# rlawhdrhs/Vision-Transformer-OpenCL

Measured on AMD Instinct MI355X. Metric: images/sec ViT-B/16 224² fp32 @batch256; % MFMA roofline; top-1 match, higher is better.
Workload: dtype f32; 1 GPU; ViT-B/16 224x224 fp32 forward, batch 256 per GPU, synthetic weights and images (BASELINE.json configs[1]); batch_per_gpu=256, global_batch=256, parallelism=dp1, lanes_per_gpu=1, prune_last_layer=False, ln_fold=True, device=AMD Radeon Graphics, arch=gfx950:sramecc+:xnack-, compute_units=256, clock_mhz=2400

## Files before the change

### vision-transformer-opencl_amd/csrc/vit_attention_hd.hip

```cpp
#include <hip/hip_runtime.h>

#include <math.h>

#include <type_traits>

#include "vit_attention.hpp"
#include "vit_hip_kernels.h"
#include "vit_split3.hpp"

namespace {

using namespace vitattn;
typedef unsigned int u32x2 __attribute__((ext_vector_type(2)));

constexpr int HD_WAVES = 4, HD_THREADS = HD_WAVES * 64;
constexpr int HD_QROWS = HD_WAVES * 32;

template <int HD, bool BF16>
struct Geo {
    typedef typename std::conditional<BF16, bf16_t, float>::type elem;
    static constexpr int VEC = BF16 ? 8 : 4;
    static constexpr int KC = BF16 ? 64 : 32;
    static constexpr int KT = KC / 32;
    static constexpr int DT = (HD + 31) / 32;
    static constexpr int HDK = BF16 ? (HD + 15) / 16 * 16 : HD;
    static constexpr int KROW = HDK + (BF16 ? 8 : 4);
    static constexpr int VROW = KC + 4;
    static constexpr int K_ELEMS = KC * KROW, V_ELEMS = DT * 32 * VROW;
    static constexpr int MIN_WAVES = BF16 && HD <= 96 ? 4 : 3;
};

template <int HD, bool BF16, bool QS>
__global__ __launch_bounds__(HD_THREADS, (Geo<HD, BF16>::MIN_WAVES)) void attention_hd_kernel(
    const typename Geo<HD, BF16>::elem *__restrict__ qkv, typename Geo<HD, BF16>::elem *__restrict__ out, int tokens, int heads, int q_rows,
    int qblocks, float scale) {
    typedef Geo<HD, BF16> G;
    typedef typename G::elem elem;
    constexpr int VEC = G::VEC, KC = G::KC, KT = G::KT, DT = G::DT, KROW = G::KROW, VROW = G::VROW;
    __shared__ __attribute__((aligned(16))) elem Ks[G::K_ELEMS];
    __shared__ __attribute__((aligned(16))) elem Vt[G::V_ELEMS];

    const int tid = threadIdx.x, lane = tid & 63, wave = tid >> 6;
    const int r = lane & 31, h = lane >> 5;
    const int image = blockIdx.x / qblocks, qblock = blockIdx.x - image * qblocks, head = blockIdx.y;
    const size_t D = (size_t)heads * HD, ld = 3 * D;
    const elem *rows = qkv + (size_t)image * tokens * ld + (size_t)head * HD;
    const elem *krows = rows + D, *vrows = rows + 2 * D;
    const int qrow0 = qblock * HD_QROWS + wave * 32;
    const bool active = qrow0 < q_rows;

    constexpr int NQ = BF16 ? G::HDK / 16 : HD / 8;
    typename std::conditional<BF16, bf16x8, f32x4>::type qf[NQ];
    {
        int qrow = qrow0 + r;
        qrow = qrow < q_rows ? qrow : q_rows - 1;
        const elem *qp = rows + (size_t)qrow * ld;
#pragma unroll
        for (int ks = 0; ks < NQ; ++ks) {
            if constexpr (BF16) {
                const int d0 = 16 * ks + 8 * h;
                u32x4 w = {0u, 0u, 0u, 0u};
                if (d0 < HD && active) w = *reinterpret_cast<const u32x4 *>(qp + d0);
                qf[ks] = __builtin_bit_cast(bf16x8, w);
            } else {
                f32x4 w = {0.0f, 0.0f, 0.0f, 0.0f};
                if (active) w = *reinterpret_cast<const f32x4 *>(qp + 8 * ks + 4 * h);
                qf[ks] = w;
            }
        }
    }

    f32x16 o[DT];
#pragma unroll
    for (int dt = 0; dt < DT; ++dt)
#pragma unroll
        for (int v = 0; v < 16; ++v) o[dt][v] = 0.0f;
    float m_run = -INFINITY, l_run = 0.0f;

    for (int key0 = 0; key0 < tokens; key0 += KC) {
        constexpr int KP = G::HDK / VEC;
        for (int i = tid; i < KC * KP; i += HD_THREADS) {
            const int row = i / KP, c = i - row * KP, key = key0 + row;
            u32x4 w = {0u, 0u, 0u, 0u};
            if (key < tokens && c * VEC < HD) w = *reinterpret_cast<const u32x4 *>(krows + (size_t)key * ld + c * VEC);
            *reinterpret_cast<u32x4 *>(Ks + row * KROW + c * VEC) = w;
        }
        constexpr int VP = HD / VEC;
        if constexpr (BF16) {
            for (int i = tid; i < (KC / 2) * VP; i += HD_THREADS) {
                const int c = i / (KC / 2), row = 2 * (i - c * (KC / 2)), key = key0 + row;
                u32x4 a = {0u, 0u, 0u, 0u}, b = {0u, 0u, 0u, 0u};
                if (key < tokens) a = *reinterpret_cast<const u32x4 *>(vrows + (size_t)key * ld + c * VEC);
                if (key + 1 < tokens) b = *reinterpret_cast<const u32x4 *>(vrows + (size_t)(key + 1) * ld + c * VEC);
#pragma unroll
                for (int j = 0; j < 4; ++j) {
                    *reinterpret_cast<unsigned *>(Vt + (c * 8 + 2 * j) * VROW + row) = (a[j] & 0xffffu) | (b[j] << 16);
                    *reinterpret_cast<unsigned *>(Vt + (c * 8 + 2 * j + 1) * VROW + row) = (a[j] >> 16) | (b[j] & 0xffff0000u);
                }
            }
        } else {
            for (int i = tid; i < KC * VP; i += HD_THREADS) {
                const int c = i / KC, row = i - c * KC, key = key0 + row;
                u32x4 w = {0u, 0u, 0u, 0u};
                if (key < tokens) w = *reinterpret_cast<const u32x4 *>(vrows + (size_t)key * ld + c * VEC);
#pragma unroll
                for (int j = 0; j < 4; ++j) Vt[(c * 4 + j) * VROW + row] = __uint_as_float(w[j]);
            }
        }
        __syncthreads();

        if (active) {
#pragma unroll
            for (int t = 0; t < KT; ++t) {
                const int tile0 = key0 + 32 * t;
                if (tile0 >= tokens) break;
                f32x16 s;
#pragma unroll
                for (int v = 0; v < 16; ++v) s[v] = 0.0f;
                const elem *kp = Ks + (32 * t + r) * KROW;
#pragma unroll
                for (int ks = 0; ks < NQ; ++ks) {
                    if constexpr (BF16) {
                        const bf16x8 kf = *reinterpret_cast<const bf16x8 *>(kp + 16 * ks + 8 * h);
                        s = __builtin_amdgcn_mfma_f32_32x32x16_bf16(kf, qf[ks], s, 0, 0, 0);
                    } else {
                        const f32x4 kf = *reinterpret_cast<const f32x4 *>(kp + 8 * ks + 4 * h);
#pragma unroll
                        for (int i = 0; i < 4; ++i) s = __builtin_amdgcn_mfma_f32_32x32x2f32(kf[i], qf[ks][i], s, 0, 0, 0);
                    }
                }
                if (tile0 + 32 > tokens) {
#pragma unroll
                    for (int v = 0; v < 16; ++v) {
                        const int key = tile0 + (v & 3) + 8 * (v >> 2) + 4 * h;
                        s[v] = key < tokens ? s[v] : -INFINITY;
                    }
                }
                float cmax = s[0];
#pragma unroll
                for (int v = 1; v < 16; ++v) cmax = fmaxf(cmax, s[v]);
                cmax = fmaxf(cmax, __shfl_xor(cmax, 32));
                constexpr float kDefer = 8.0f;
                const float m_old = m_run;
                const float m_new = (cmax - m_old) * scale > kDefer ? cmax : m_old;
                const float mneg = -m_new * scale;
                m_run = m_new;
                float sum = 0.0f;
#pragma unroll
                for (int v = 0; v < 16; ++v) {
                    s[v] = __builtin_amdgcn_exp2f(QS ? s[v] + mneg : fmaf(s[v], scale, mneg));
                    sum += s[v];
                }
                if (__any(m_new != m_old)) {
                    const float alpha = __builtin_amdgcn_exp2f((m_old - m_new) * scale);
                    l_run *= alpha;
#pragma unroll
                    for (int dt = 0; dt < DT; ++dt)
#pragma unroll
                        for (int v = 0; v < 16; ++v) o[dt][v] *= alpha;
                }
                l_run += sum;
                if constexpr (BF16) {
#pragma unroll
                    for (int s2 = 0; s2 < 2; ++s2) {
                        bf16x8 pf, pl;
#pragma unroll
                        for (int j = 0; j < 8; ++j) {
                            pf[j] = (__bf16)s[8 * s2 + j];
                            pl[j] = (__bf16)(s[8 * s2 + j] - (float)pf[j]);
                        }
#pragma unroll
                        for (int dt = 0; dt < DT; ++dt) {
                            const bf16_t *vp = Vt + (32 * dt + r) * VROW + 32 * t + 16 * s2 + 4 * h;
                            const u32x2 lo = *reinterpret_cast<const u32x2 *>(vp), hi = *reinterpret_cast<const u32x2 *>(vp + 8);
                            const u32x4 both = {lo[0], lo[1], hi[0], hi[1]};
                            o[dt] = __builtin_amdgcn_mfma_f32_32x32x16_bf16(__builtin_bit_cast(bf16x8, both), pl, o[dt], 0, 0, 0);
                            o[dt] = __builtin_amdgcn_mfma_f32_32x32x16_bf16(__builtin_bit_cast(bf16x8, both), pf, o[dt], 0, 0, 0);
                        }
                    }
                } else {
#pragma unroll
                    for (int q = 0; q < 4; ++q)
#pragma unroll
                        for (int dt = 0; dt < DT; ++dt) {
                            const f32x4 vf = *reinterpret_cast<const f32x4 *>(Vt + (32 * dt + r) * VROW + 32 * t + 8 * q + 4 * h);
#pragma unroll
                            for (int i = 0; i < 4; ++i) o[dt] = __builtin_amdgcn_mfma_f32_32x32x2f32(vf[i], s[4 * q + i], o[dt], 0, 0, 0);
                        }
                }
            }
        }
        __syncthreads();
    }

    const int qrow = qrow0 + r;
    if (active && qrow < q_rows) {
        const float inv = 1.0f / (l_run + __shfl_xor(l_run, 32));
        elem *dst = out + ((size_t)image * tokens + qrow) * D + (size_t)head * HD;
#pragma unroll
        for (int dt = 0; dt < DT; ++dt)
#pragma unroll
            for (int q = 0; q < 4; ++q) {
                const int d0 = 32 * dt + 8 * q + 4 * h;
                if (d0 < HD) {
                    if constexpr (BF16) {
                        bf16x4 w;
#pragma unroll
                        for (int i = 0; i < 4; ++i) w[i] = (__bf16)(o[dt][4 * q + i] * inv);
                        *reinterpret_cast<u32x2 *>(dst + d0) = __builtin_bit_cast(u32x2, w);
                    } else {
                        const f32x4 w = {o[dt][4 * q] * inv, o[dt][4 * q + 1] * inv, o[dt][4 * q + 2] * inv, o[dt][4 * q + 3] * inv};
                        *reinterpret_cast<f32x4 *>(dst + d0) = w;
                    }
                }
            }
    }
}

#ifndef ATT_SPLIT_WAVES
#define ATT_SPLIT_WAVES 4
#endif
#ifndef ATT_SPLIT_MINW
#define ATT_SPLIT_MINW 3
#endif
constexpr int SP_WAVES = ATT_SPLIT_WAVES, SP_THREADS = SP_WAVES * 64, SP_QROWS = SP_WAVES * 32;

__global__ __launch_bounds__(SP_THREADS, ATT_SPLIT_MINW) void attention_split_kernel(const float *__restrict__ qkv, float *__restrict__ out,
                                                                                    int tokens, int heads, int q_rows, int qblocks) {
    using vitsplit::SPLIT_TERM_A;
    using vitsplit::SPLIT_TERM_W;
    using vitsplit::split3_piece8;
    typedef Geo<64, true> G;
    constexpr int HD = 64, KC = G::KC, KT = G::KT, DT = G::DT, KROW = G::KROW, VROW = G::VROW, NQ = HD / 16;
    __shared__ __attribute__((aligned(16))) bf16_t Ks[3 * G::K_ELEMS];
    __shared__ __attribute__((aligned(16))) bf16_t Vt[3 * G::V_ELEMS];

    const int tid = threadIdx.x, lane = tid & 63, wave = tid >> 6;
    const int r = lane & 31, h = lane >> 5;
    const int image = blockIdx.x / qblocks, qblock = blockIdx.x - image * qblocks, head = blockIdx.y;
    const size_t D = (size_t)heads * HD, ld = 3 * D;
    const float *rows = qkv + (size_t)image * tokens * ld + (size_t)head * HD;
    const float *krows = rows + D, *vrows = rows + 2 * D;
    const int qrow0 = qblock * SP_QROWS + wave * 32;
    const bool active = qrow0 < q_rows;
    const f32x4 zero4 = {0.0f, 0.0f, 0.0f, 0.0f};

    bf16x8 qf[3][NQ];
    {
        int qrow = qrow0 + r;
        qrow = qrow < q_rows ? qrow : q_rows - 1;
        const float *qp = rows + (size_t)qrow * ld + 8 * h;
#pragma unroll
        for (int ks = 0; ks < NQ; ++ks) {
            f32x4 x0 = zero4, x1 = zero4;
            if (active) {
                x0 = *reinterpret_cast<const f32x4 *>(qp + 16 * ks);
                x1 = *reinterpret_cast<const f32x4 *>(qp + 16 * ks + 4);
            }
#pragma unroll
            for (int pl = 0; pl < 3; ++pl) qf[pl][ks] = __builtin_bit_cast(bf16x8, split3_piece8(x0, x1, pl));
        }
    }

    f32x16 o[DT];
#pragma unroll
    for (int dt = 0; dt < DT; ++dt)
#pragma unroll
        for (int v = 0; v < 16; ++v) o[dt][v] = 0.0f;
    float m_run = -INFINITY, l_run = 0.0f;

    constexpr int K_ITEMS = KC * (HD / 8), V_ITEMS = (KC / 2) * (HD / 8);
    constexpr int KI = (K_ITEMS + SP_THREADS - 1) / SP_THREADS;
    constexpr int V_TID0 = SP_THREADS > V_ITEMS ? SP_THREADS - V_ITEMS : 0;
    static_assert(V_ITEMS <= SP_THREADS, "one V item per thread at most");
    const int vi = tid - V_TID0;
    f32x4 kx[KI][2], vx[4];
    auto fetch = [&](int key0) {
#pragma unroll
        for (int it = 0; it < KI; ++it) {
            const int i = tid + it * SP_THREADS, row = i / (HD / 8), c = i - row * (HD / 8), key = key0 + row;
            kx[it][0] = kx[it][1] = zero4;
            if (i < K_ITEMS && key < tokens) {
                const float *p = krows + (size_t)key * ld + 8 * c;
                kx[it][0] = *reinterpret_cast<const f32x4 *>(p);
                kx[it][1] = *reinterpret_cast<const f32x4 *>(p + 4);
            }
        }
        if (vi >= 0) {
            const int c = vi / (KC / 2), key = key0 + 2 * (vi - c * (KC / 2));
#pragma unroll
            for (int j = 0; j < 4; ++j) vx[j] = zero4;
            if (key < tokens) {
                const float *p = vrows + (size_t)key * ld + 8 * c;
                vx[0] = *reinterpret_cast<const f32x4 *>(p);
                vx[1] = *reinterpret_cast<const f32x4 *>(p + 4);
            }
            if (key + 1 < tokens) {
                const float *p = vrows + (size_t)(key + 1) * ld + 8 * c;
                vx[2] = *reinterpret_cast<const f32x4 *>(p);
                vx[3] = *reinterpret_cast<const f32x4 *>(p + 4);
            }
        }
    };
    auto store = [&](bf16_t *Kd, bf16_t *Vd) {
#pragma unroll
        for (int it = 0; it < KI; ++it) {
            const int i = tid + it * SP_THREADS, row = i / (HD / 8), c = i - row * (HD / 8);
            if (i < K_ITEMS) {
#pragma unroll
                for (int pl = 0; pl < 3; ++pl)
                    *reinterpret_cast<u32x4 *>(Kd + pl * G::K_ELEMS + row * KROW + 8 * c) = split3_piece8(kx[it][0], kx[it][1], pl);
            }
        }
        if (vi >= 0) {
            const int c = vi / (KC / 2), row = 2 * (vi - c * (KC / 2));
#pragma unroll
            for (int pl = 0; pl < 3; ++pl) {
                const u32x4 a = split3_piece8(vx[0], vx[1], pl), b = split3_piece8(vx[2], vx[3], pl);
                bf16_t *vd = Vd + pl * G::V_ELEMS + (c * 8) * VROW + row;
#pragma unroll
                for (int j = 0; j < 4; ++j) {
                    *reinterpret_cast<unsigned *>(vd + (2 * j) * VROW) = (a[j] & 0xffffu) | (b[j] << 16);
                    *reinterpret_cast<unsigned *>(vd + (2 * j + 1) * VROW) = (a[j] >> 16) | (b[j] & 0xffff0000u);
                }
            }
        }
    };

    for (int key0 = 0; key0 < tokens; key0 += KC) {
        fetch(key0);
        store(Ks, Vt);
        __syncthreads();

        if (active) {
#pragma unroll
            for (int t = 0; t < KT; ++t) {
                const int tile0 = key0 + 32 * t;
                if (tile0 >= tokens) break;
                f32x16 s;
#pragma unroll
                for (int v = 0; v < 16; ++v) s[v] = 0.0f;
                const bf16_t *kp = Ks + (32 * t + r) * KROW + 8 * h;
#pragma unroll
                for (int ks = 0; ks < NQ; ++ks) {
                    bf16x8 kf[3];
#pragma unroll
                    for (int pl = 0; pl < 3; ++pl) kf[pl] = *reinterpret_cast<const bf16x8 *>(kp + pl * G::K_ELEMS + 16 * ks);
#pragma unroll
                    for (int term = 0; term < 6; ++term)
                        s = __builtin_amdgcn_mfma_f32_32x32x16_bf16(kf[SPLIT_TERM_A[term]], qf[SPLIT_TERM_W[term]][ks], s, 0, 0, 0);
                }
                if (tile0 + 32 > tokens) {
#pragma unroll
                    for (int v = 0; v < 16; ++v) {
                        const int key = tile0 + (v & 3) + 8 * (v >> 2) + 4 * h;
                        s[v] = key < tokens ? s[v] : -INFINITY;
                    }
                }
                float cmax = s[0];
#pragma unroll
                for (int v = 1; v < 16; ++v) cmax = fmaxf(cmax, s[v]);
                cmax = fmaxf(cmax, __shfl_xor(cmax, 32));
                constexpr float kDefer = 8.0f, scale = kScale64;
                const float m_old = m_run;
                const float m_new = (cmax - m_old) * scale > kDefer ? cmax : m_old;
                const float mneg = -m_new * scale;
                m_run = m_new;
                float sum = 0.0f;
#pragma unroll
                for (int v = 0; v < 16; ++v) {
                    s[v] = __builtin_amdgcn_exp2f(fmaf(s[v], scale, mneg));
                    sum += s[v];
                }
                if (__any(m_new != m_old)) {
                    const float alpha = __builtin_amdgcn_exp2f((m_old - m_new) * scale);
                    l_run *= alpha;
#pragma unroll
                    for (int dt = 0; dt < DT; ++dt)
#pragma unroll
                        for (int v = 0; v < 16; ++v) o[dt][v] *= alpha;
                }
                l_run += sum;
#pragma unroll
                for (int s2 = 0; s2 < 2; ++s2) {
                    if (tile0 + 16 * s2 >= tokens) break;
                    f32x4 x0 = {s[8 * s2], s[8 * s2 + 1], s[8 * s2 + 2], s[8 * s2 + 3]};
                    f32x4 x1 = {s[8 * s2 + 4], s[8 * s2 + 5], s[8 * s2 + 6], s[8 * s2 + 7]};
                    bf16x8 pf[3], vf[DT][3];
#pragma unroll
                    for (int pl = 0; pl < 3; ++pl) pf[pl] = __builtin_bit_cast(bf16x8, split3_piece8(x0, x1, pl));
#pragma unroll
                    for (int dt = 0; dt < DT; ++dt)
#pragma unroll
                        for (int pl = 0; pl < 3; ++pl) {
                            const bf16_t *vp = Vt + pl * G::V_ELEMS + (32 * dt + r) * VROW + 32 * t + 16 * s2 + 4 * h;
                            const u32x2 lo = *reinterpret_cast<const u32x2 *>(vp), hi = *reinterpret_cast<const u32x2 *>(vp + 8);
                            const u32x4 both = {lo[0], lo[1], hi[0], hi[1]};
                            vf[dt][pl] = __builtin_bit_cast(bf16x8, both);
                        }
#pragma unroll
                    for (int term = 0; term < 6; ++term)
#pragma unroll
                        for (int dt = 0; dt < DT; ++dt)
                            o[dt] = __builtin_amdgcn_mfma_f32_32x32x16_bf16(vf[dt][SPLIT_TERM_A[term]], pf[SPLIT_TERM_W[term]], o[dt], 0, 0, 0);
                }
            }
        }
        __syncthreads();
    }

    const int qrow = qrow0 + r;
    if (active && qrow < q_rows) {
        const float inv = 1.0f / (l_run + __shfl_xor(l_run, 32));
        float *dst = out + ((size_t)image * tokens + qrow) * D + (size_t)head * HD + 4 * h;
#pragma unroll
        for (int dt = 0; dt < DT; ++dt)
#pragma unroll
            for (int q = 0; q < 4; ++q) {
                const f32x4 w = {o[dt][4 * q] * inv, o[dt][4 * q + 1] * inv, o[dt][4 * q + 2] * inv, o[dt][4 * q + 3] * inv};
                *reinterpret_cast<f32x4 *>(dst + 32 * dt + 8 * q) = w;
            }
    }
}

template <bool BF16, bool QS>
int launch_hd(hipStream_t s, const typename Geo<128, BF16>::elem *qkv, typename Geo<128, BF16>::elem *out, int n_images, int tokens,
              int heads, int head_dim, int q_rows) {
    const int qblocks = (q_rows + HD_QROWS - 1) / HD_QROWS;
    if (heads > 65535 || (long long)n_images * qblocks > 0x7fffffffLL) return static_cast<int>(hipErrorInvalidValue);
    const float scale = QS ? 1.0f : vithip_qscale(head_dim);
    return dispatch_int<72, 8, 8>(head_dim, [&](auto hd) {
        hipLaunchKernelGGL((attention_hd_kernel<decltype(hd)::value, BF16, QS>), dim3((unsigned)(n_images * qblocks), (unsigned)heads),
                           dim3(HD_THREADS), 0, s, qkv, out, tokens, heads, q_rows, qblocks, scale);
        return static_cast<int>(hipGetLastError());
    });
}

}

int vitattn::attention_hd_f32(hipStream_t s, const float *qkv, float *out, int n_images, int tokens, int heads, int head_dim, int q_rows) {
    return launch_hd<false, false>(s, qkv, out, n_images, tokens, heads, head_dim, q_rows);
}

int vitattn::attention_hd_bf16(hipStream_t s, const unsigned short *qkv, unsigned short *out, int n_images, int tokens, int heads,
                               int head_dim, int q_rows, bool q_scaled) {
    return q_scaled ? launch_hd<true, true>(s, qkv, out, n_images, tokens, heads, head_dim, q_rows)
                    : launch_hd<true, false>(s, qkv, out, n_images, tokens, heads, head_dim, q_rows);
}

int vitattn::attention_split_f32(hipStream_t s, const float *qkv, float *out, int n_images, int tokens, int heads, int q_rows) {
    const int qblocks = (q_rows + SP_QROWS - 1) / SP_QROWS;
    if (heads > 65535 || (long long)n_images * qblocks > 0x7fffffffLL) return static_cast<int>(hipErrorInvalidValue);
    hipLaunchKernelGGL(attention_split_kernel, dim3((unsigned)(n_images * qblocks), (unsigned)heads), dim3(SP_THREADS), 0, s, qkv, out,
                       tokens, heads, q_rows, qblocks);
    return static_cast<int>(hipGetLastError());
}

extern "C" float vithip_qscale(int head_dim) {
    if (!vitattn::hd_accepted(head_dim)) return 0.0f;
    return (float)((1.0 / sqrt((double)head_dim)) * 1.4426950408889634074);
}
```

Measured before the change: 5964 images/sec.

## Stage V row-major with transposed LDS reads and zero-fill padded key tiles

The split-bf16 attention kernel now stores V in LDS row-major, with an XOR swizzle, using the same per-thread staging as K. It builds the PV MFMA operand through a transpose-read helper (v_fragment_tr) instead of scattering 16-bit transposed writes at store time. Padded key rows past the token count are written as zeros without splitting the loaded values, and the wave index is made wave-uniform with readfirstlane. This is meant to cut LDS store cost and bank conflicts during staging, in exchange for a different V read pattern and a static LDS-capacity check against the occupancy target.

```diff
diff --git a/vision-transformer-opencl_amd/csrc/vit_attention_hd.hip b/vision-transformer-opencl_amd/csrc/vit_attention_hd.hip
--- a/vision-transformer-opencl_amd/csrc/vit_attention_hd.hip
+++ b/vision-transformer-opencl_amd/csrc/vit_attention_hd.hip
@@ -223,7 +223,17 @@
 #ifndef ATT_SPLIT_MINW
 #define ATT_SPLIT_MINW 3
 #endif
+#ifndef ATT_SPLIT_VTR
+#define ATT_SPLIT_VTR 1
+#endif
+#ifndef ATT_SPLIT_PADSKIP
+#define ATT_SPLIT_PADSKIP 1
+#endif
 constexpr int SP_WAVES = ATT_SPLIT_WAVES, SP_THREADS = SP_WAVES * 64, SP_QROWS = SP_WAVES * 32;
+constexpr int SP_VROW = ATT_SPLIT_VTR ? 64 : Geo<64, true>::VROW;
+constexpr int SP_V_ELEMS = ATT_SPLIT_VTR ? Geo<64, true>::KC * SP_VROW : Geo<64, true>::V_ELEMS;
+constexpr int SP_LDS_BYTES = 3 * (Geo<64, true>::K_ELEMS + SP_V_ELEMS) * (int)sizeof(bf16_t);
+static_assert(ATT_SPLIT_MINW * 4 / SP_WAVES * SP_LDS_BYTES <= 160 * 1024, "the workgroups the launch bounds ask for share one CU's LDS");
 
 __global__ __launch_bounds__(SP_THREADS, ATT_SPLIT_MINW) void attention_split_kernel(const float *__restrict__ qkv, float *__restrict__ out,
                                                                                     int tokens, int heads, int q_rows, int qblocks) {
@@ -231,11 +241,11 @@
     using vitsplit::SPLIT_TERM_W;
     using vitsplit::split3_piece8;
     typedef Geo<64, true> G;
-    constexpr int HD = 64, KC = G::KC, KT = G::KT, DT = G::DT, KROW = G::KROW, VROW = G::VROW, NQ = HD / 16;
+    constexpr int HD = 64, KC = G::KC, KT = G::KT, DT = G::DT, KROW = G::KROW, VROW = SP_VROW, NQ = HD / 16;
     __shared__ __attribute__((aligned(16))) bf16_t Ks[3 * G::K_ELEMS];
-    __shared__ __attribute__((aligned(16))) bf16_t Vt[3 * G::V_ELEMS];
-
-    const int tid = threadIdx.x, lane = tid & 63, wave = tid >> 6;
+    __shared__ __attribute__((aligned(16))) bf16_t Vt[3 * SP_V_ELEMS];
+
+    const int tid = threadIdx.x, lane = tid & 63, wave = __builtin_amdgcn_readfirstlane(tid >> 6);
     const int r = lane & 31, h = lane >> 5;
     const int image = blockIdx.x / qblocks, qblock = blockIdx.x - image * qblocks, head = blockIdx.y;
     const size_t D = (size_t)heads * HD, ld = 3 * D;
@@ -269,8 +279,46 @@
         for (int v = 0; v < 16; ++v) o[dt][v] = 0.0f;
     float m_run = -INFINITY, l_run = 0.0f;
 
-    constexpr int K_ITEMS = KC * (HD / 8), V_ITEMS = (KC / 2) * (HD / 8);
-    constexpr int KI = (K_ITEMS + SP_THREADS - 1) / SP_THREADS;
+    constexpr int ITEMS = KC * (HD / 8), NI = ITEMS / SP_THREADS;
+    static_assert(ITEMS % SP_THREADS == 0, "every thread stages the same number of items");
+#if ATT_SPLIT_VTR
+    f32x4 kx[NI][2], vx[NI][2];
+    auto fetch = [&](int key0) {
+#pragma unroll
+        for (int it = 0; it < NI; ++it) {
+            const int i = tid + it * SP_THREADS, row = i / (HD / 8), c = i - row * (HD / 8), key = key0 + row;
+            kx[it][0] = kx[it][1] = vx[it][0] = vx[it][1] = zero4;
+            if (key < tokens) {
+                const float *kp = krows + (size_t)key * ld + 8 * c, *vp = vrows + (size_t)key * ld + 8 * c;
+                kx[it][0] = *reinterpret_cast<const f32x4 *>(kp);
+                kx[it][1] = *reinterpret_cast<const f32x4 *>(kp + 4);
+                vx[it][0] = *reinterpret_cast<const f32x4 *>(vp);
+                vx[it][1] = *reinterpret_cast<const f32x4 *>(vp + 4);
+            }
+        }
+    };
+    auto store = [&](int key0) {
+#pragma unroll
+        for (int it = 0; it < NI; ++it) {
+            const int i = tid + it * SP_THREADS, row = i / (HD / 8), c = i - row * (HD / 8);
+            bf16_t *kd = Ks + row * KROW + 8 * c, *vd = Vt + row * VROW + 8 * (c ^ (4 * ((row >> 1) & 1)));
+            if (ATT_SPLIT_PADSKIP && key0 + 8 * wave + it * (SP_THREADS / 8) >= tokens) {
+#pragma unroll
+                for (int pl = 0; pl < 3; ++pl) {
+                    *reinterpret_cast<u32x4 *>(kd + pl * G::K_ELEMS) = u32x4{0u, 0u, 0u, 0u};
+                    *reinterpret_cast<u32x4 *>(vd + pl * SP_V_ELEMS) = u32x4{0u, 0u, 0u, 0u};
+                }
+            } else {
+#pragma unroll
+                for (int pl = 0; pl < 3; ++pl) {
+                    *reinterpret_cast<u32x4 *>(kd + pl * G::K_ELEMS) = split3_piece8(kx[it][0], kx[it][1], pl);
+                    *reinterpret_cast<u32x4 *>(vd + pl * SP_V_ELEMS) = split3_piece8(vx[it][0], vx[it][1], pl);
+                }
+            }
+        }
+    };
+#else
+    constexpr int K_ITEMS = ITEMS, V_ITEMS = (KC / 2) * (HD / 8), KI = NI;
     constexpr int V_TID0 = SP_THREADS > V_ITEMS ? SP_THREADS - V_ITEMS : 0;
     static_assert(V_ITEMS <= SP_THREADS, "one V item per thread at most");
     const int vi = tid - V_TID0;
@@ -302,34 +350,45 @@
             }
         }
     };
-    auto store = [&](bf16_t *Kd, bf16_t *Vd) {
+    auto store = [&](int key0) {
 #pragma unroll
         for (int it = 0; it < KI; ++it) {
             const int i = tid + it * SP_THREADS, row = i / (HD / 8), c = i - row * (HD / 8);
-            if (i < K_ITEMS) {
+            if (ATT_SPLIT_PADSKIP && key0 + 8 * wave + it * (SP_THREADS / 8) >= tokens) {
+#pragma unroll
+                for (int pl = 0; pl < 3; ++pl) *reinterpret_cast<u32x4 *>(Ks + pl * G::K_ELEMS + row * KROW + 8 * c) = u32x4{0u, 0u, 0u, 0u};
+            } else {
 #pragma unroll
                 for (int pl = 0; pl < 3; ++pl)
-                    *reinterpret_cast<u32x4 *>(Kd + pl * G::K_ELEMS + row * KROW + 8 * c) = split3_piece8(kx[it][0], kx[it][1], pl);
+                    *reinterpret_cast<u32x4 *>(Ks + pl * G::K_ELEMS + row * KROW + 8 * c) = split3_piece8(kx[it][0], kx[it][1], pl);
             }
         }
         if (vi >= 0) {
             const int c = vi / (KC / 2), row = 2 * (vi - c * (KC / 2));
-#pragma unroll
-            for (int pl = 0; pl < 3; ++pl) {
-                const u32x4 a = split3_piece8(vx[0], vx[1], pl), b = split3_piece8(vx[2], vx[3], pl);
-                bf16_t *vd = Vd + pl * G::V_ELEMS + (c * 8) * VROW + row;
-#pragma unroll
-                for (int j = 0; j < 4; ++j) {
-                    *reinterpret_cast<unsigned *>(vd + (2 * j) * VROW) = (a[j] & 0xffffu) | (b[j] << 16);
-                    *reinterpret_cast<unsigned *>(vd + (2 * j + 1) * VROW) = (a[j] >> 16) | (b[j] & 0xffff0000u);
+            if (ATT_SPLIT_PADSKIP && key0 + row >= tokens) {
+#pragma unroll
+                for (int pl = 0; pl < 3; ++pl)
+#pragma unroll
+                    for (int j = 0; j < 8; ++j) *reinterpret_cast<unsigned *>(Vt + pl * SP_V_ELEMS + (c * 8 + j) * VROW + row) = 0u;
+            } else {
+#pragma unroll
+                for (int pl = 0; pl < 3; ++pl) {
+                    const u32x4 a = split3_piece8(vx[0], vx[1], pl), b = split3_piece8(vx[2], vx[3], pl);
+                    bf16_t *vd = Vt + pl * SP_V_ELEMS + (c * 8) * VROW + row;
+#pragma unroll
+                    for (int j = 0; j < 4; ++j) {
+                        *reinterpret_cast<unsigned *>(vd + (2 * j) * VROW) = (a[j] & 0xffffu) | (b[j] << 16);
+                        *reinterpret_cast<unsigned *>(vd + (2 * j + 1) * VROW) = (a[j] >> 16) | (b[j] & 0xffff0000u);
+                    }
                 }
             }
         }
     };
+#endif
 
     for (int key0 = 0; key0 < tokens; key0 += KC) {
         fetch(key0);
-        store(Ks, Vt);
+        store(key0);
         __syncthreads();
 
         if (active) {
@@ -393,10 +452,14 @@
                     for (int dt = 0; dt < DT; ++dt)
 #pragma unroll
                         for (int pl = 0; pl < 3; ++pl) {
-                            const bf16_t *vp = Vt + pl * G::V_ELEMS + (32 * dt + r) * VROW + 32 * t + 16 * s2 + 4 * h;
+#if ATT_SPLIT_VTR
+                            vf[dt][pl] = v_fragment_tr<VROW>(Vt + pl * SP_V_ELEMS, 32 * t + 16 * s2, dt, lane);
+#else
+                            const bf16_t *vp = Vt + pl * SP_V_ELEMS + (32 * dt + r) * VROW + 32 * t + 16 * s2 + 4 * h;
                             const u32x2 lo = *reinterpret_cast<const u32x2 *>(vp), hi = *reinterpret_cast<const u32x2 *>(vp + 8);
                             const u32x4 both = {lo[0], lo[1], hi[0], hi[1]};
                             vf[dt][pl] = __builtin_bit_cast(bf16x8, both);
+#endif
                         }
 #pragma unroll
                     for (int term = 0; term < 6; ++term)
```

New measurement: 5996 images/sec, median of 6. Within noise of the previous version (+0.5%).
